# wusize/CLIPSelf

Measured on AMD Instinct MI355X. Metric: images/sec (student+teacher distill step), ViT-B/16 32 crops/img, higher is better.
Workload: dtype bf16; 1 GPU; EVA02-CLIP-B-16 CLIPSelf image-patches step, 64 images x 32 crops per GPU, 224^2 (BASELINE configs[1]); global_batch=64, crops_per_image=32, image_size=224, parallelism=dp1, teacher_chunk=2048, teacher_last_block=cls_query_only, teacher_schedule=one_batch_ahead_on_side_stream

## Files before the change

clipself_amd/csrc/attention.hip:

```cpp
#include <type_traits>
#include "cs_common.h"
#include "../../include/clipself_hip.h"
#include <cstdlib>

namespace {

constexpr int HD = 64;
constexpr float LOG2E = 1.4426950408889634f;


#define Z16 (f32x16{0.f, 0.f, 0.f, 0.f, 0.f, 0.f, 0.f, 0.f, 0.f, 0.f, 0.f, 0.f, 0.f, 0.f, 0.f, 0.f})
__device__ __forceinline__ f32x16 zero16() {
    f32x16 z;
#pragma unroll
    for (int e = 0; e < 16; ++e) z[e] = 0.f;
    return z;
}

__device__ __forceinline__ void rope8(U128& v, const float* __restrict__ cs, const float* __restrict__ sn) {
    const float4 c0 = *(const float4*)cs, c1 = *(const float4*)(cs + 4);
    const float4 s0 = *(const float4*)sn, s1 = *(const float4*)(sn + 4);
    const float c[8] = {c0.x, c0.y, c0.z, c0.w, c1.x, c1.y, c1.z, c1.w};
    const float s[8] = {s0.x, s0.y, s0.z, s0.w, s1.x, s1.y, s1.z, s1.w};
#pragma unroll
// ... 373 lines not shown
    constexpr int KI = (CHK * 8 + NT - 1) / NT;
    U128 kr[KI], vin[8], qraw[4];
    const __bf16* kbase = p.qkv + C + h * HD;
    const __bf16* vbase = p.qkv + 2 * C + h * HD;
    const int vkb = min(tid, CHK - 1) >> 3, vc = tid & 7;
#pragma unroll
    for (int it = 0; it < KI; ++it) {
        const int idx = min(tid + it * NT, CHK * 8 - 1), tok = min(idx >> 3, last);
        kr[it].u = *(const uint4*)(kbase + (rowbase + tok) * p.ldqkv + (idx & 7) * 8);
    }
#pragma unroll
    for (int i = 0; i < 8; ++i) {
        const int tok = min(vkb * 8 + i, last);
        vin[i].u = *(const uint4*)(vbase + (rowbase + tok) * p.ldqkv + vc * 8);
    }
    const int q0 = wave * 32, q = q0 + l31, qc = min(q, last);
#pragma unroll
    for (int ks = 0; ks < 4; ++ks) qraw[ks].u = *(const uint4*)(p.qkv + (rowbase + qc) * p.ldqkv + h * HD + ks * 16 + hf * 8);
    if constexpr (ROPE) {
        if (tid < p.grid * 32) {
            rt[tid] = tab[0];
            rt[(p.grid << 5) + tid] = tab[1];
            rt[(2 * p.grid << 5) + tid] = tab[2];
            rt[(3 * p.grid << 5) + tid] = tab[3];
        }
        __syncthreads();
    }
#pragma unroll
    for (int it = 0; it < KI; ++it) {
        const int idx = tid + it * NT, r = idx >> 3, c = idx & 7;
        if (idx < CHK * 8) {
// ... 19 lines not shown
        if (ROPE && qc > 0 && !ATT_ABL(p, 2)) rope8_lds(qraw[ks], rt, p.grid, p.inv_grid, qc, ks * 2 + hf);
        qf[ks] = qraw[ks].h;
    }
    float m = -INFINITY, l = 0.f;
    f32x16 o[2] = {zero16(), zero16()};
    if (ATT_ABL(p, 1)) { l = 1.f; m = 0.f; o[0][0] = bf2f(qf[0][0]); }
    else if (TAIL) {
        attend_chunk<3, false, false, !ROPE>(Kl, Vt, qf, 0, p.Ntok, sl2, lane, true, m, l, o, 0);
        attend_chunk<3, false, false, !ROPE>(Kl, Vt, qf, 96, p.Ntok, sl2, lane, false, m, l, o, 3);
        attend_chunk<1, true, false, !ROPE>(Kl, Vt, qf, 192, p.Ntok, sl2, lane, false, m, l, o, 6);
    } else {
        attend_chunk<3, false>(Kl, Vt, qf, 0, p.Ntok, sl2, lane, true, m, l, o, 0);
        if (p.Ntok > 96) attend_chunk<3, false>(Kl, Vt, qf, 96, p.Ntok, sl2, lane, false, m, l, o, 3);
        if (p.Ntok > 192) attend_chunk<1, false>(Kl, Vt, qf, 192, p.Ntok, sl2, lane, false, m, l, o, 6);
    }
    if (q < p.Ntok) store_o(p, rowbase, q, h, bh, hf, m, l, o);
}

__global__ __launch_bounds__(256) void attn_bwd_prep_kernel(const __bf16* __restrict__ o, const __bf16* __restrict__ dout, float* __restrict__ dsum,
                                                            int B, int Ntok, int H, int ldo) {
    const long idx = (long)blockIdx.x * blockDim.x + threadIdx.x;
    const long total = (long)B * Ntok * H * 8;
    float s = 0.f;
    long row = 0; int h = 0;
    const bool ok = idx < total;
    if (ok) {
        const int c = (int)(idx & 7);
        h = (int)((idx >> 3) % H);
        row = (idx >> 3) / H;
        U128 a, g;
        a.u = *(const uint4*)(o + row * ldo + h * HD + c * 8);
// ... 1091 lines not shown
```

clipself_amd/csrc/gemm.hip:

```cpp
#include "gemm_common.h"
#include "../../include/clipself_hip.h"
#include <hip/amd_detail/amd_hip_unsafe_atomics.h>

namespace {

constexpr int EP_LD = 68;
constexpr int EP_BYTES = 32 * EP_LD * 4;

template <int FM, int BN>
__device__ __forceinline__ void epilogue_swiglu(const GemmArgs& p, const f32x16 (&acc)[FM][2], char* slab_bytes, char* rowst_bytes, int lane,
                                                int row0, int tn, int wn) {
    const int l31 = lane & 31, hf = lane >> 5;
    uint32_t* slab = (uint32_t*)slab_bytes;
    const int hbase = tn * (BN / 2) + wn * 32;
    const int hl = hbase + l31;
    float b1 = 0.f, b2 = 0.f;
    if (p.bias && hl < p.group) { b1 = p.bias[hl]; b2 = p.bias[p.group + hl]; }
    const bool ln = p.ln_mean != nullptr;
    float c1 = 0.f, c2 = 0.f;
    float2* rowst = (float2*)rowst_bytes;
    if (ln) {
        if (hl < p.group) { c1 = p.ln_colsum[hl]; c2 = p.ln_colsum[p.group + hl]; }
        for (int r = lane; r < FM * 32; r += 64) {
            const int row = min(row0 + r, p.M - 1);
// ... 262 lines not shown
                for (int it = 0; it < 8; ++it) {
                    const float a = sum_lanes16(ps[it]), b = sum_lanes16(pq[it]);
                    if (sel == it) { sv = a; qv = b; }
                }
                const int row = row_base + rrow + 4 * sel;
                if (sel < 8 && row < p.M && n0 + wn * 64 < p.N) {
                    const size_t slice = (size_t)tn * (BN / 64) + wn;
                    *(float2*)(p.stats_part + (slice * p.M + row) * 2) = make_float2(sv, qv);
                }
            }
        }
        if (i + 1 < FM) asm volatile("s_waitcnt lgkmcnt(0)" ::: "memory");
    }
}

template <int EPI, int BM, int BN, int WM, int WN, bool GLDS, int NS>
__global__ __launch_bounds__(WM * WN * 64) void gemm_nt_kernel(GemmArgs p) {
    constexpr int NW = WM * WN;
    constexpr int TM = BM / WM, TN = BN / WN;
    constexpr int FM = TM / 32, FN = TN / 32;
    constexpr int A_BYTES = BM * BK * 2, B_BYTES = BN * BK * 2, STAGE = A_BYTES + B_BYTES;
    constexpr int A_INSTR = BM / 8 / NW, B_INSTR = BN / 8 / NW;
    extern __shared__ __attribute__((aligned(16))) char smem[];

    const int tid = threadIdx.x;
    const int lane = tid & 63;
    const int wave = __builtin_amdgcn_readfirstlane(tid >> 6);
    const int wm = wave / WN, wn = wave - wm * WN;
    const int hf = lane >> 5, l31 = lane & 31;
    int tm, tn;
    tile_of_block(p, tm, tn);
    const int m0 = tm * BM, n0 = tn * BN;

    int arow[A_INSTR], achk[A_INSTR], brow[B_INSTR], bchk[B_INSTR];
    source_rows<EPI, BM, BN, NW, A_INSTR, B_INSTR>(p, wave, lane, m0, n0, tn, arow, achk, brow, bchk);

    const int kt_begin = blockIdx.y * p.ktiles_per_split;
    const int kt_end = min(kt_begin + p.ktiles_per_split, p.K / BK);

    f32x16 acc[FM][FN];
#pragma unroll
    for (int i = 0; i < FM; ++i)
#pragma unroll
        for (int j = 0; j < FN; ++j)
#pragma unroll
            for (int e = 0; e < 16; ++e) acc[i][j][e] = 0.f;

    constexpr bool AB = (NS == 32);
    char* const b_ring = smem + 3 * A_BYTES;
    if (kt_begin < kt_end) {
        stage_tile<A_INSTR, GLDS>(p.A, p.lda, kt_begin * BK, smem, wave * A_INSTR, lane, arow, achk);
        stage_tile<B_INSTR, GLDS>(p.B, p.ldb, kt_begin * BK, AB ? b_ring : smem + A_BYTES, wave * B_INSTR, lane, brow, bchk);
    }
    if (AB && kt_begin + 1 < kt_end)
        stage_tile<A_INSTR, GLDS>(p.A, p.lda, (kt_begin + 1) * BK, smem + A_BYTES, wave * A_INSTR, lane, arow, achk);
    const int a_base = ((wm * TM + l31) >> 1) << 8;
    const int b_base = ((wn * TN + l31) >> 1) << 8;
    const int par8 = (l31 & 1) << 3, sw = l31 >> 1;
    int cur = 0;
    for (int kt = kt_begin; kt < kt_end; ++kt) {
        if (AB) {
            if (kt + 1 < kt_end) asm volatile("s_waitcnt vmcnt(%0)" ::"n"(A_INSTR) : "memory");
            else asm volatile("s_waitcnt vmcnt(0)" ::: "memory");
            asm volatile("s_waitcnt lgkmcnt(0)" ::: "memory");
            __builtin_amdgcn_s_barrier();
            const int i = kt - kt_begin;
            if (!(A_INSTR == 4 && B_INSTR == 4) || (p.dbg & 8)) {
                if (kt + 1 < kt_end)
                    stage_tile<B_INSTR, GLDS>(p.B, p.ldb, (kt + 1) * BK, b_ring + ((i + 1) & 1) * B_BYTES, wave * B_INSTR, lane, brow, bchk);
                if (kt + 2 < kt_end)
                    stage_tile<A_INSTR, GLDS>(p.A, p.lda, (kt + 2) * BK, smem + ((i + 2) % 3) * A_BYTES, wave * A_INSTR, lane, arow, achk);
            }
        } else {
            __syncthreads();
            if (kt + 1 < kt_end && !CS_ABL(p, 1)) {
                char* nxt = smem + (cur ^ 1) * STAGE;
                stage_tile<A_INSTR, GLDS>(p.A, p.lda, (kt + 1) * BK, nxt, wave * A_INSTR, lane, arow, achk);
                stage_tile<B_INSTR, GLDS>(p.B, p.ldb, (kt + 1) * BK, nxt + A_BYTES, wave * B_INSTR, lane, brow, bchk);
            }
        }
        const char* la = (AB ? smem + cur * A_BYTES : smem + cur * STAGE) + a_base;
        const char* lb = (AB ? b_ring + ((kt - kt_begin) & 1) * B_BYTES : smem + cur * STAGE + A_BYTES) + b_base;
        if (CS_ABL(p, 2)) { cur = AB ? (cur == 2 ? 0 : cur + 1) : (cur ^ 1); continue; }
#pragma unroll
        for (int ks = 0; ks < 4; ++ks) {
            const int off = ((par8 | (ks * 2 + hf)) ^ sw) << 4;
            bf16x8 a[FM], b[FN];
#pragma unroll
            for (int i = 0; i < FM; ++i) a[i] = *(const bf16x8*)(la + i * (16 * 256) + off);
#pragma unroll
            for (int j = 0; j < FN; ++j) b[j] = *(const bf16x8*)(lb + j * (16 * 256) + off);
            if (AB && A_INSTR == 4 && B_INSTR == 4 && !(p.dbg & 8)) {
                const int i0 = kt - kt_begin;
#pragma unroll
                for (int h2 = 0; h2 < 2; ++h2) {
                    const int x = (ks & 1) * 2 + h2;
                    if (ks < 2) {
                        if (kt + 1 < kt_end) {
                            const int r1[1] = {brow[x]}, c1[1] = {bchk[x]};
                            stage_tile<1, GLDS>(p.B, p.ldb, (kt + 1) * BK, b_ring + ((i0 + 1) & 1) * B_BYTES, wave * B_INSTR + x, lane, r1, c1);
                        }
                    } else if (kt + 2 < kt_end) {
                        const int r1[1] = {arow[x]}, c1[1] = {achk[x]};
                        stage_tile<1, GLDS>(p.A, p.lda, (kt + 2) * BK, smem + ((i0 + 2) % 3) * A_BYTES, wave * A_INSTR + x, lane, r1, c1);
                    }
                }
            }
#pragma unroll
            for (int i = 0; i < FM; ++i)
#pragma unroll
                for (int j = 0; j < FN; ++j) acc[i][j] = __builtin_amdgcn_mfma_f32_32x32x16_bf16(a[i], b[j], acc[i][j], 0, 0, 0);
        }
        cur = AB ? (cur == 2 ? 0 : cur + 1) : (cur ^ 1);
    }
    __syncthreads();
    if (CS_ABL(p, 4)) return;
    epilogue<EPI, FM, FN, BN>(p, acc, smem, wave, lane, m0 + wm * TM, n0, tn, wn);
}

template <int EPI, int RM = 0>
__global__ __launch_bounds__(512) void gemm_persist_kernel(GemmArgs p) {
    constexpr int AUX_A = RM == 2 ? 2 : 0, AUX_B = RM == 3 ? 2 : 0;
    constexpr bool BSTAT = RM == 1 || RM == 2;
    static_assert(epi_is_bf16(EPI) || EPI == EPI_SWIGLU_BF16 || EPI == EPI_RESID_F32 || EPI == EPI_RESID_LN_F32, "epilogues whose slabs fit");
    constexpr bool PACKED = epi_is_bf16(EPI) || EPI == EPI_SWIGLU_BF16;
    constexpr int BM = 256, BN = 256, WN = 4, NW = 8, TM = 128, TN = 64, FM = 4, FN = 2;
// ... 80 lines not shown
            if (more) tile_of_id(p, next, ntiles, tm, tn);
        }
        if (more) {
            source_rows<EPI, BM, BN, NW, A_INSTR, B_INSTR>(p, wave, lane, tm * BM, tn * BN, tn, arow, achk, brow, bchk);
            prologue();
        }
        if constexpr (EPI == EPI_SWIGLU_BF16) epilogue_swiglu<FM, BN>(p, acc, slab, rowst, lane, m0 + wm * TM, tn_cur, wn);
        else if constexpr (epi_is_bf16(EPI)) epilogue_bf16<FM, BN, epi_act(EPI)>(p, acc, slab, rowst, lane, m0 + wm * TM, n0, wn);
        else epilogue_at<EPI, FM, FN, BN, 64>(p, acc, slab, lane, m0 + wm * TM, n0, tn_cur, wn);
        if (!more) break;
        tile = next;
        first = false;
    }
}

template <int EPI, int BM, int BN, int WM, int WN, int NS>
int launch_cfg(GemmArgs a, int splits, int use_glds, hipStream_t stream) {
    a.tiles_m = (a.M + BM - 1) / BM;
    a.tiles_n = (EPI == EPI_SWIGLU_BF16) ? (a.group + BN / 2 - 1) / (BN / 2) : (a.N + BN - 1) / BN;
    constexpr int NW = WM * WN;
    constexpr size_t stage = NS == 32 ? (size_t)(3 * BM + 2 * BN) * BK * 2 : (size_t)(BM + BN) * BK * 2 * NS;
    constexpr size_t lds = stage > (size_t)NW * EP_BYTES ? stage : (size_t)NW * EP_BYTES;
    dim3 grid(a.tiles_m * a.tiles_n, splits), block(NW * 64);
    if (use_glds) {
        static bool once = ((void)hipFuncSetAttribute((const void*)gemm_nt_kernel<EPI, BM, BN, WM, WN, true, NS>,
                                                      hipFuncAttributeMaxDynamicSharedMemorySize, (int)lds), true);
        (void)once;
        hipLaunchKernelGGL((gemm_nt_kernel<EPI, BM, BN, WM, WN, true, NS>), grid, block, lds, stream, a);
    } else {
        static bool once = ((void)hipFuncSetAttribute((const void*)gemm_nt_kernel<EPI, BM, BN, WM, WN, false, NS>,
                                                      hipFuncAttributeMaxDynamicSharedMemorySize, (int)lds), true);
        (void)once;
        hipLaunchKernelGGL((gemm_nt_kernel<EPI, BM, BN, WM, WN, false, NS>), grid, block, lds, stream, a);
    }
    CS_LAUNCH_CHECK();
    return 0;
}

template <int EPI, int RM>
// ... 11 lines not shown
    constexpr int BM = 256, BN = 256;
    a.tiles_m = (a.M + BM - 1) / BM;
    a.tiles_n = (EPI == EPI_SWIGLU_BF16) ? (a.group + BN / 2 - 1) / (BN / 2) : (a.N + BN - 1) / BN;
    const long ntiles = (long)a.tiles_m * a.tiles_n;
    const long cap = cs_persistent_cap(a.reserve);
    const unsigned grid = (unsigned)(ntiles < cap ? ntiles : cap);
    if constexpr (EPI == EPI_BF16 || EPI == EPI_SWIGLU_BF16) {
        const bool parts_ok = (long)grid == cap && grid % 8 == 0 && a.tiles_n >= a.nsplit && a.tiles_m >= 8 / a.nsplit;
        if (a.rm == 1 && parts_ok) return launch_persist_rm<EPI, 1>(a, grid, stream);
        if (a.rm == 2 && parts_ok) return launch_persist_rm<EPI, 2>(a, grid, stream);
        if (a.rm == 3) return launch_persist_rm<EPI, 3>(a, grid, stream);
    }
    return launch_persist_rm<EPI, 0>(a, grid, stream);
}

template <int EPI>
int launch(GemmArgs a, int splits, int use_glds, int force_cfg, hipStream_t stream) {
    const long ncols = (EPI == EPI_SWIGLU_BF16) ? 2L * a.group : a.N;
    const int ktiles = a.K / BK;
    auto tiles = [&](int bm, int bn) { return (long)((a.M + bm - 1) / bm) * ((ncols + bn - 1) / bn); };
    const double out_bytes = 4.0 * (double)a.M * (double)ncols;
    auto best_split = [&](int bm, int bn, int per_cu, double us_per_ktile, double& cost) {
        const long t = tiles(bm, bn);
        const long slots = (long)cs_num_cus() * per_cu;
        int best = 1;
        cost = 1e30;
        const int lo = splits > 0 ? splits : 1, hi = splits > 0 ? splits : (ktiles < 64 ? ktiles : 64);
        for (int s = lo; s <= hi; ++s) {
            const long rounds = (t * s + slots - 1) / slots;
            const int kper = (ktiles + s - 1) / s;
            const double c = rounds * (kper * us_per_ktile + 5.0) + (EPI == EPI_ATOMIC_F32 ? s * out_bytes / 0.33e6 : 0.0);
            if (c < cost) { cost = c; best = s; }
        }
        return best;
    };
    double c1, c2, c3;
    const int sp[4] = {0, best_split(128, 128, 2, 1.3, c1), best_split(256, 128, 1, 0.95, c2), best_split(256, 256, 1, 1.4, c3)};
    int cfg = force_cfg;
    if (cfg == 0) {
        if (a.M < 256 || ncols < 256) c3 = 1e30;
        if (a.M < 256 || ncols < 128) c2 = 1e30;
        cfg = (c3 <= c2 && c3 <= c1) ? 3 : (c2 <= c1 ? 2 : 1);
        if (cfg == 3 && use_glds) cfg = 11;
    }
    if (cfg != 1 && cfg != 2 && cfg != 3 && cfg != 7 && cfg != 9 && cfg != 11) {
        cs_set_error("cs_gemm_nt: schedule %d does not exist (flags bits 4-7: 0 heuristic, 1, 2, 3, 7, 9, 11)", cfg);
        return -1;
    }
    const int ns = sp[cfg >= 7 ? 3 : cfg];
    a.ktiles_per_split = (ktiles + ns - 1) / ns;
    if (cfg == 11) {
        if (use_glds && ns == 1) {
            const int rc = cs_gemm_stream_launch(a, EPI, a.reserve, stream);
            if (rc <= 0) return rc;
        }
        cfg = 9;
    }
    switch (cfg) {
        case 9:
            if constexpr (epi_is_bf16(EPI) || EPI == EPI_SWIGLU_BF16 || EPI == EPI_RESID_F32 || EPI == EPI_RESID_LN_F32) {
                if (use_glds && ns == 1) return launch_persist<EPI>(a, stream);
            }
            return launch_cfg<EPI, 256, 256, 2, 4, 32>(a, ns, use_glds, stream);
        case 7: return launch_cfg<EPI, 256, 256, 2, 4, 32>(a, ns, use_glds, stream);
        case 3: return launch_cfg<EPI, 256, 256, 2, 4, 2>(a, ns, use_glds, stream);
        case 2: return launch_cfg<EPI, 256, 128, 4, 2, 2>(a, ns, use_glds, stream);
        default: return launch_cfg<EPI, 128, 128, 2, 2, 2>(a, ns, use_glds, stream);
    }
}

__global__ __launch_bounds__(256) void splitk_reduce_act_kernel(const float* __restrict__ ws, int splits, long stride,
                                                                const float* __restrict__ bias, __bf16* __restrict__ C, int M, int N,
                                                                int ldc, int relu) {
    const long i = (long)blockIdx.x * 256 + threadIdx.x;
    const int n4 = N >> 2;
    if (i >= (long)M * n4) return;
    const int row = (int)(i / n4), c = (int)(i - (long)row * n4) * 4;
    const float* src = ws + (size_t)row * N + c;
    float4 acc = *(const float4*)src;
    for (int s = 1; s < splits; ++s) {
        const float4 t = *(const float4*)(src + (size_t)s * stride);
        acc.x += t.x; acc.y += t.y; acc.z += t.z; acc.w += t.w;
// ... 10 lines not shown
}

constexpr int SPLITK_MAX = 8, SPLITK_MIN_KTILES = 16;
int choose_bf16_splits(int M, int N, int K) {
    const long tiles = (long)((M + 255) / 256) * ((N + 255) / 256);
    const int ktiles = K / BK;
    int s = 1;
    while (s < SPLITK_MAX && tiles * (s * 2) <= cs_num_cus() && ktiles / (s * 2) >= SPLITK_MIN_KTILES) s *= 2;
    return s;
}

}

static int gemm_nt_split_f32(const void* A, const void* B, float* C, int M, int N, int K, int lda, int ldb, int cfg, int splits, hipStream_t stream);

static int gemm_nt_impl(const void* A, const void* B, void* C, const float* bias, const float* extra, const float* ln_mean,
                        const float* ln_rstd, const float* ln_colsum, float* stats_part, void* xb_out, int ldxb, int M, int N, int K, int lda,
                        int ldb, int ldc, int epi, int splits, int group, int flags, hipStream_t stream) {
    if (epi == EPI_THIN_FWD || epi == EPI_THIN_DGRAD) {
        CS_CHECK_ARG(!ln_mean && !ln_rstd && !ln_colsum && !stats_part && !xb_out, "cs_gemm_nt_ln: epilogue %d takes no folded LayerNorm", epi);
        return cs_thin_launch(A, B, C, bias, extra, M, N, K, lda, ldb, ldc, epi, splits, group, flags, stream);
    }
    CS_CHECK_ARG(M > 0 && N > 0 && K > 0, "cs_gemm_nt: empty problem M=%d N=%d K=%d", M, N, K);
    CS_CHECK_ARG(K % BK == 0, "cs_gemm_nt: K=%d must be a multiple of %d", K, BK);
    CS_CHECK_ARG((lda % 8) == 0 && (ldb % 8) == 0, "cs_gemm_nt: lda/ldb must be multiples of 8 (16-byte rows)");
    CS_CHECK_ARG(((uintptr_t)A % 16) == 0 && ((uintptr_t)B % 16) == 0, "cs_gemm_nt: operands must be 16-byte aligned");
    const bool splitk_bf16 = (epi == EPI_BF16 || epi == EPI_RELU_BF16) && ln_mean == nullptr;
    CS_CHECK_ARG(splits == 1 || epi == EPI_ATOMIC_F32 || splitk_bf16,
                 "cs_gemm_nt: split-K (splits != 1; <= 0 = automatic) exists for epilogues 0 and 9 (through a workspace) and 4 (atomic), not %d", epi);
    CS_CHECK_ARG((epi == EPI_SWIGLU_BF16 ? group : N) % 4 == 0 && ldc % 4 == 0 && ((uintptr_t)C % 16) == 0,
                 "cs_gemm_nt: N, ldc must be multiples of 4 and C 16-byte aligned (vector epilogue)");
    CS_CHECK_ARG(bias == nullptr || ((uintptr_t)bias % 16) == 0, "cs_gemm_nt: bias must be 16-byte aligned");
    if (splitk_bf16 && splits != 1) {
        const int ns = splits > 0 ? splits : choose_bf16_splits(M, N, K);
        CS_CHECK_ARG(ns <= K / BK, "cs_gemm_nt: splits=%d exceeds the %d K tiles of K=%d", ns, K / BK, K);
        if (ns > 1) {
// ... 325 lines not shown
```

clipself_amd/csrc/gemm_common.h:

```cpp
#pragma once
#include "cs_common.h"
#include <cstdio>
#include <cstdlib>
#include <type_traits>

#ifdef CS_ABLATION_SWITCHES
#define CS_ABL(p, bit) ((p).dbg & (bit))
#else
#define CS_ABL(p, bit) false
#endif

constexpr int BK = 64;
enum Epi { EPI_BF16 = 0, EPI_F32 = 1, EPI_RESID_F32 = 2, EPI_SWIGLU_BF16 = 3, EPI_ATOMIC_F32 = 4, EPI_PATCH_F32 = 5, EPI_RESID_LN_F32 = 6,
           EPI_GELU_BF16 = 7, EPI_QGELU_BF16 = 8, EPI_RELU_BF16 = 9, EPI_THIN_FWD = 10, EPI_THIN_DGRAD = 11 };
constexpr bool epi_is_bf16(int e) { return e == EPI_BF16 || e == EPI_GELU_BF16 || e == EPI_QGELU_BF16 || e == EPI_RELU_BF16; }
constexpr int epi_act(int e) { return e == EPI_GELU_BF16 ? 1 : (e == EPI_QGELU_BF16 ? 2 : (e == EPI_RELU_BF16 ? 3 : 0)); }

struct GemmArgs {
    const __bf16* A;
    const __bf16* B;
    void* C;
    const float* bias;
    const float* extra;
    int M, N, K;
    int lda, ldb, ldc;
    int tiles_m, tiles_n;
    int ktiles_per_split;
    long split_stride;
    int group;
    int gm;
    int rm;
    int nsplit;
    const float* ln_mean;
    const float* ln_rstd;
    const float* ln_colsum;
    float* stats_part;
    __bf16* xb_out;
    int ldxb;
    unsigned short* lo = nullptr;
    int split = 0;
    int reserve;
    int dbg;
};

inline int cs_num_cus() {
    static const int n = [] {
        int dev = 0, v = 0;
        if (hipGetDevice(&dev) != hipSuccess || hipDeviceGetAttribute(&v, hipDeviceAttributeMultiprocessorCount, dev) != hipSuccess || v <= 0) v = 256;
        return v;
    }();
    return n;
}
inline long cs_persistent_cap(int reserve) {
    const int n = cs_num_cus();
    return n - (reserve > 0 && reserve <= n - 8 ? reserve : 0);
// ... 80 lines not shown
```

clipself_amd/engine.py:

```python
from __future__ import annotations

import math
import os

import torch

from .config import TowerCfg
from .engine_base import (ALIGN, BF16, DX_BF16, DX_F32_ACCUM, DX_F32_ASSIGN, EPI_ATOMIC_F32, EPI_BF16, EPI_F32, EPI_GELU_BF16,
                          EPI_PATCH_F32, EPI_QGELU_BF16, EPI_RESID_F32, EPI_RESID_LN_F32, EPI_SWIGLU_BF16, F32, TowerEngine, _round_up,
                          is_no_decay, padded_hidden)


def param_groups_layout(cfg: TowerCfg, prefix: str = "visual."):
    C, Hd, E, p = cfg.width, cfg.hidden, cfg.embed_dim, cfg.patch_size
    Hp, Kp = padded_hidden(cfg), _round_up(3 * p * p, 64)
    t = lambda name, shape, storage=None: (name, shape, storage if storage is not None else shape)
    groups = [[t(prefix + "cls_token", (1, 1, C))], [t(prefix + "pos_embed", (1, cfg.tokens, C))],
              [t(prefix + "patch_embed.proj.weight", (C, 3, p, p), (C, Kp))], [t(prefix + "patch_embed.proj.bias", (C,))]]
    for i in range(cfg.layers):
        b = f"{prefix}{EvaEngine.BLOCK_TAG}{i}."
        groups += [
            [t(b + "norm1.weight", (C,))], [t(b + "norm1.bias", (C,))],
            [t(b + "attn.q_proj.weight", (C, C)), t(b + "attn.k_proj.weight", (C, C)), t(b + "attn.v_proj.weight", (C, C))],
            [t(b + "attn.q_bias", (C,)), t(b + "attn._k_bias_zero", (C,)), t(b + "attn.v_bias", (C,))],
# ... 172 lines not shown
            half = self.cfg.head_width // 2
            freqs = 1.0 / (10000.0 ** (torch.arange(0, half, 2)[: half // 2].float() / half))
            t = torch.arange(grid).float() / grid * self.cfg.pt_hw_seq_len
            ang = (t[:, None] * freqs[None, :]).repeat_interleave(2, dim=-1)
            full = torch.cat([ang[:, None, :].expand(grid, grid, half), ang[None, :, :].expand(grid, grid, half)], dim=-1)
            full = full.reshape(grid * grid, self.cfg.head_width)
            self._tables[key] = (full.cos().contiguous().to(self.device), full.sin().contiguous().to(self.device))
        return self._tables[key]

    def _stem(self, images, keep=None):
        ops, cfg, P = self.ops, self.cfg, self.prefix
        B, _, S, _ = images.shape
        p, C = cfg.patch_size, cfg.width
        g = S // p
        N, Kpe = g * g + 1, self.Kpe
        A = ops.empty((B * g * g, Kpe), BF16)
        ops.im2row(images.contiguous(), A, p)
        x = ops.empty((B, N, C), F32)
        pos = self.pos_for(g)
        ops.gemm_nt(A, self.storage_of(self.shadow, P + "patch_embed.proj.weight"), x.view(B * N, C),
                    bias=self.p[P + "patch_embed.proj.bias"], extra=pos, epi=EPI_PATCH_F32, group=g * g)
        ops.cls_row(x, self.p[P + "cls_token"].view(C), pos)
        if keep is not None:
            keep["patches"] = A
        return x, g

    def _stacked(self, buf, name, i):
        o, st = self.offsets[self._b(i) + name]
        n = self.STACKED[name]
        return buf[o:o + n * math.prod(st)].view(n * st[0], *st[1:])

    def _qkv_operands(self, i):
        return self._stacked(self.shadow, "attn.q_proj.weight", i), self._stacked(self.master, "attn.q_bias", i)

    def _w12(self, i):
        return self._stacked(self.shadow, "mlp.w1.weight", i), self._stacked(self.master, "mlp.w1.bias", i)

    def _block_linears(self, i):
        b = self._b(i)
# ... 185 lines not shown
```

clipself_amd/engine_base.py:

```python
from __future__ import annotations

import math
import os
from collections import OrderedDict

import torch
import torch.nn.functional as F

from .config import TowerCfg

BF16, F32 = torch.bfloat16, torch.float32
EPI_BF16, EPI_F32, EPI_RESID_F32, EPI_SWIGLU_BF16, EPI_ATOMIC_F32, EPI_PATCH_F32, EPI_RESID_LN_F32, EPI_GELU_BF16, EPI_QGELU_BF16 = range(9)
DX_BF16, DX_F32_ASSIGN, DX_F32_ACCUM = range(3)
ALIGN = 64


def _round_up(x: int, m: int) -> int:
    return (x + m - 1) // m * m


def padded_hidden(cfg: TowerCfg) -> int:
    return _round_up(cfg.hidden, 64)


# ... 109 lines not shown
        self.sync_shadow()
        return missing

    def sync_shadow(self):
        self.ops.cast_f32_bf16(self.master, self.shadow)
        self._pos_cache.clear()
        self.block_fold_ratio = None
        if self.trainable or self.HEAD_FWD_TRANSPOSED:
            self.sync_transposed()
        if self._wants_folds():
            self._build_folds()

    def _wants_folds(self) -> bool:
        return self.fold_block_ln

    def _wt_alloc(self, key, rows, cols):
        t = self.wt.get(key)
        if t is None:
            t = self.ops.zeros((cols, _round_up(rows, 64)), BF16)
            self.wt[key] = t
        return t

    def _block_wt_pairs(self, blocks=None):
        blocks = range(self.first_trainable, self.cfg.layers) if blocks is None else blocks
        return [(W, self._wt_alloc((i, key), *W.shape)) for i in blocks for key, W in self._block_linears(i)]

    def set_trainable_blocks(self, unlocked_groups: int):
        L = self.cfg.layers
        self.first_trainable = L - unlocked_groups if 0 < unlocked_groups <= L else 0
        self.train_all = False
# ... 428 lines not shown
```

clipself_amd/engine_openai.py:

```python
from __future__ import annotations

import os

import torch

from .config import TowerCfg
from .engine_base import (BF16, DX_F32_ACCUM, DX_F32_ASSIGN, EPI_BF16, EPI_F32, EPI_GELU_BF16, EPI_PATCH_F32, EPI_QGELU_BF16,
                          EPI_RESID_F32, F32, TowerEngine, _round_up)


def clip_vit_layout(cfg: TowerCfg, prefix: str = "visual."):
    C, Hd, E, p = cfg.width, cfg.hidden, cfg.embed_dim, cfg.patch_size
    Kp = _round_up(3 * p * p, 64)
    t = lambda name, shape, storage=None: (name, shape, storage if storage is not None else shape)
    groups = [[t(prefix + "class_embedding", (C,))], [t(prefix + "positional_embedding", (cfg.tokens, C))],
              [t(prefix + "conv1.weight", (C, 3, p, p), (C, Kp))], [t(prefix + "ln_pre.weight", (C,))], [t(prefix + "ln_pre.bias", (C,))]]
    for i in range(cfg.layers):
        b = f"{prefix}{ClipVitEngine.BLOCK_TAG}{i}."
        groups += [[t(b + "ln_1.weight", (C,))], [t(b + "ln_1.bias", (C,))],
                   [t(b + "attn.in_proj_weight", (3 * C, C))], [t(b + "attn.in_proj_bias", (3 * C,))],
                   [t(b + "attn.out_proj.weight", (C, C))], [t(b + "attn.out_proj.bias", (C,))],
                   [t(b + "ln_2.weight", (C,))], [t(b + "ln_2.bias", (C,))],
                   [t(b + "mlp.c_fc.weight", (Hd, C))], [t(b + "mlp.c_fc.bias", (Hd,))],
                   [t(b + "mlp.c_proj.weight", (C, Hd))], [t(b + "mlp.c_proj.bias", (C,))]]
# ... 118 lines not shown
    def rope_tables(self, grid: int):
        if getattr(self.ops, "ATTN_NO_ROPE", False) and os.environ.get("CLIPSELF_ATTN_IDENTITY_ROPE", "0") in ("", "0"):
            return None, None
        key = ("rope", grid)
        if key not in self._tables:
            shape = (grid * grid, self.cfg.head_width)
            self._tables[key] = (torch.ones(shape, dtype=F32, device=self.device), torch.zeros(shape, dtype=F32, device=self.device))
        return self._tables[key]

    def _stem(self, images, keep=None):
        ops, cfg, P = self.ops, self.cfg, self.prefix
        B, _, S, _ = images.shape
        p, C = cfg.patch_size, cfg.width
        g = S // p
        N = g * g + 1
        A = ops.empty((B * g * g, self.Kpe), BF16)
        ops.im2row(images.contiguous(), A, p)
        x = ops.empty((B, N, C), F32)
        pos = self.pos_for(g)
        ops.gemm_nt(A, self.storage_of(self.shadow, P + "conv1.weight"), x.view(B * N, C), extra=pos, epi=EPI_PATCH_F32, group=g * g)
        ops.cls_row(x, self.p[P + "class_embedding"], pos)
        y = ops.empty((B, N, C), F32)
        mean = rstd = None
        if keep is not None:
            mean, rstd = ops.empty((B * N,), F32), ops.empty((B * N,), F32)
            keep.update(patches=A, x_pre=x.view(B * N, C), st=(mean, rstd))
        ops.layernorm_fwd_f32(x.view(B * N, C), self.p[P + "ln_pre.weight"], self.p[P + "ln_pre.bias"], y.view(B * N, C), mean, rstd, cfg.ln_eps)
        return y, g

    def _block_tail(self, i, x, att, save=None, inplace=True):
        return block_fwd_mlp(self.ops, self.p, self.w, self._b(i), self.cfg.ln_eps, self.cfg.quick_gelu, x, att, save, inplace)

    def _block_fwd(self, i, x, B, N, cos, sin, with_attn=True, save=None, inplace=True):
        ops, cfg = self.ops, self.cfg
        C, H, eps = cfg.width, cfg.heads, cfg.ln_eps
# ... 258 lines not shown
```

clipself_amd/hip.py:

```python
from __future__ import annotations

import ctypes
import os
import subprocess
from pathlib import Path

import torch

_CSRC = Path(__file__).resolve().parent / "csrc"
_LIB_PATH = Path(os.environ["CLIPSELF_HIP_LIB"]) if os.environ.get("CLIPSELF_HIP_LIB") else _CSRC / "libclipself_hip.so"

EPI_BF16, EPI_F32, EPI_RESID_F32, EPI_SWIGLU_BF16, EPI_ATOMIC_F32, EPI_PATCH_F32, EPI_RESID_LN_F32, EPI_GELU_BF16, EPI_QGELU_BF16 = range(9)
EPI_RELU_BF16 = 9
EPI_THIN_FWD, EPI_THIN_DGRAD = 10, 11
THIN_MAX_N = 16
SPLITK_MAX, SPLITK_MIN_KTILES = 8, 16
DX_BF16, DX_F32_ASSIGN, DX_F32_ACCUM = range(3)
ADAMW_GUARD_HEAD, ADAMW_GUARD_SPAN = 8, 16384

_vp, _i, _l, _f, _sz = ctypes.c_void_p, ctypes.c_int, ctypes.c_long, ctypes.c_float, ctypes.c_size_t
_F32, _F32_BF16 = (torch.float32,), (torch.float32, torch.bfloat16)

SIGNATURES = {
    "cs_last_error": (ctypes.c_char_p, []),
    "cs_gemm_nt": (_i, [_vp, _vp, _vp, _vp, _vp, _i, _i, _i, _i, _i, _i, _i, _i, _i, _i, _vp]),
    "cs_crop_resize_workspace": (_sz, [_i, _i, _i]),
    "cs_crop_resize_u8": (_i, [_vp, _i, _i, _vp, _i, _i, _i, _vp, _vp, _vp, _vp, _vp]),
    "cs_quant_rows_fp8": (_i, [_vp, _l, _vp, _l, _vp, _i, _i, _vp]),
    "cs_gemm_nt_f8": (_i, [_vp, _vp, _vp, _vp, _vp, _vp, _vp, _i, _i, _i, _i, _i, _i, _i, _i, _vp]),
# ... 207 lines not shown
    ADAMW_GUARD = True
    ATTN_NO_ROPE = True
    TOKEN_TAPS = True
    DECONV_ROWS = True
    DET_POST = True
    ROI_EXTRACT = True
    ASSIGN = True
    LOSS = True
    MASK = True
    RPN = True
    CONV3X3 = True
    BATCHNORM = True
    LINEAR_ACT = True
    FPN_TOPDOWN = True
    THIN_HEADS = True
    BOX_SCORES = True

    def __init__(self):
        self.lib = load_library()
        if not torch.cuda.is_available():
            raise RuntimeError("HipOps needs a ROCm device (torch.cuda.is_available() is False); no CPU fallback exists")
        self.gemm_flags = 0
        self._rccl_reserve = 0
        self._share = 0
        self._cap = 0
        self.num_cus = int(self.lib.cs_num_compute_units())

    def _update_flags(self):
        n = self._rccl_reserve + self._share
        if self._cap:
# ... 558 lines not shown

    def colsum_bf16(self, x, out, workspace=None):
        self._chk(x, out, workspace)
        M, N = x.shape
        need = self.colsum_workspace(M, N)
        if workspace is None or workspace.numel() * workspace.element_size() < need:
            workspace = torch.empty(need, dtype=torch.uint8, device=x.device)
        self._ok(self.lib.cs_colsum_bf16(_p(x), x.stride(0), _p(out), _p(workspace), M, N, self._stream()), "cs_colsum_bf16")

    def im2row(self, img, out, p):
        self._chk(img, out)
        B, _, S, _ = img.shape
        assert img.is_contiguous()
        assert out.stride(1) == 1 and out.stride(0) == out.shape[1], "im2row writes whole rows (zeros in [3*p*p, ldo)): out must be contiguous"
        self._ok(self.lib.cs_im2row(_p(img), _dt(img), _p(out), B, S, p, out.stride(0), self._stream()), "cs_im2row")

    def cls_row(self, x, cls, pos):
        self._chk(x, cls, pos)
        B, Ntok, C = x.shape
        self._ok(self.lib.cs_cls_row(_p(x), _p(cls), _p(pos), B, Ntok, C, self._stream()), "cs_cls_row")

    @staticmethod
    def _token_map(feat, grid_h, grid_w, tok_off):
        E = feat.shape[-1]
        assert feat.dtype == torch.float32 and feat.stride(-1) == 1 and E % 4 == 0 and feat.stride(0) % E == 0 and feat.data_ptr() % 16 == 0
        if feat.dim() == 4:
            assert tuple(feat.shape[1:3]) == (grid_h, grid_w) and feat.stride(2) == E and feat.stride(1) == grid_w * E, \
                "a [B, h, w, E] map must be a view of the token-major layout"
        else:
            assert feat.dim() == 3 and feat.stride(1) == E
# ... 605 lines not shown
```

Baseline: 749.2 images/sec.

## Fuse im2row into patch-embed GEMM via implicit image A-operand loads

The patch-embedding GEMM now gathers its A operand straight from the image tensor (fp32 or bf16), rounds it to bf16 in registers and writes it to LDS. This replaces the separate im2row kernel and its materialised bf16 patch matrix whenever backward does not need the patches kept. It removes one kernel launch and a round trip of the patch matrix through memory, but A now goes through register loads instead of the DMA path and forgoes schedule 11. A separate change adds an ablation flag to the attention kernel that makes one wave recompute queries redundantly without storing them.

```diff
diff --git a/clipself_amd/csrc/attention.hip b/clipself_amd/csrc/attention.hip
--- a/clipself_amd/csrc/attention.hip
+++ b/clipself_amd/csrc/attention.hip
@@ -411,7 +411,8 @@
         const int tok = min(vkb * 8 + i, last);
         vin[i].u = *(const uint4*)(vbase + (rowbase + tok) * p.ldqkv + vc * 8);
     }
-    const int q0 = wave * 32, q = q0 + l31, qc = min(q, last);
+    const bool redundant = ATT_ABL(p, 8) && wave == 7;
+    const int q0 = redundant ? 0 : wave * 32, q = q0 + l31, qc = min(q, last);
 #pragma unroll
     for (int ks = 0; ks < 4; ++ks) qraw[ks].u = *(const uint4*)(p.qkv + (rowbase + qc) * p.ldqkv + h * HD + ks * 16 + hf * 8);
     if constexpr (ROPE) {
@@ -461,7 +462,7 @@
         if (p.Ntok > 96) attend_chunk<3, false>(Kl, Vt, qf, 96, p.Ntok, sl2, lane, false, m, l, o, 3);
         if (p.Ntok > 192) attend_chunk<1, false>(Kl, Vt, qf, 192, p.Ntok, sl2, lane, false, m, l, o, 6);
     }
-    if (q < p.Ntok) store_o(p, rowbase, q, h, bh, hf, m, l, o);
+    if (q < p.Ntok && !redundant) store_o(p, rowbase, q, h, bh, hf, m, l, o);
 }
 
 __global__ __launch_bounds__(256) void attn_bwd_prep_kernel(const __bf16* __restrict__ o, const __bf16* __restrict__ dout, float* __restrict__ dsum,
diff --git a/clipself_amd/csrc/gemm.hip b/clipself_amd/csrc/gemm.hip
--- a/clipself_amd/csrc/gemm.hip
+++ b/clipself_amd/csrc/gemm.hip
@@ -300,8 +300,52 @@
     }
 }
 
-template <int EPI, int BM, int BN, int WM, int WN, bool GLDS, int NS>
+template <int IMG>
+struct PatchRun {
+    uint4 v[IMG == 1 ? 2 : 1];
+};
+
+__device__ __forceinline__ int patch_row_base(const GemmArgs& p, int row, int img0) {
+    const int b = row / p.group, t = row - b * p.group;
+    const int py = t / p.img_g, px = t - py * p.img_g;
+    return (((b - img0) * 3 * p.lda + (py << p.img_lp)) * p.lda) + (px << p.img_lp);
+}
+
+template <int IMG>
+__device__ __forceinline__ void patch_fetch(const GemmArgs& p, const void* img, int base, int k, bool live, PatchRun<IMG>& r) {
+    const int pm = (1 << p.img_lp) - 1;
+    const int c = k >> (2 * p.img_lp), iy = (k >> p.img_lp) & pm, ix = k & pm;
+    const int off = live ? base + (c * p.lda + iy) * p.lda + ix : 0;
+    if (IMG == 1) {
+        const uint4* s = (const uint4*)((const float*)img + off);
+        r.v[0] = s[0];
+        r.v[1] = s[1];
+    } else {
+        r.v[0] = *(const uint4*)((const __bf16*)img + off);
+    }
+}
+
+template <int IMG>
+__device__ __forceinline__ uint4 patch_round(const PatchRun<IMG>& r) {
+    U128 o;
+    if (IMG == 1) {
+        union { uint4 u[2]; float f[8]; } s;
+        s.u[0] = r.v[0];
+        s.u[1] = r.v[1];
+#pragma unroll
+        for (int e = 0; e < 8; ++e) o.e[e] = f2bf(s.f[e]);
+    } else {
+        U128 s;
+        s.u = r.v[0];
+#pragma unroll
+        for (int e = 0; e < 8; ++e) o.e[e] = f2bf((float)s.e[e]);
+    }
+    return o.u;
+}
+
+template <int EPI, int BM, int BN, int WM, int WN, bool GLDS, int NS, int IMG = 0>
 __global__ __launch_bounds__(WM * WN * 64) void gemm_nt_kernel(GemmArgs p) {
+    static_assert(IMG == 0 || (EPI == EPI_PATCH_F32 && GLDS), "the implicit A operand belongs to the patch embedding; B keeps the DMA");
     constexpr int NW = WM * WN;
     constexpr int TM = BM / WM, TN = BN / WN;
     constexpr int FM = TM / 32, FN = TN / 32;
@@ -320,6 +364,23 @@
 
     int arow[A_INSTR], achk[A_INSTR], brow[B_INSTR], bchk[B_INSTR];
     source_rows<EPI, BM, BN, NW, A_INSTR, B_INSTR>(p, wave, lane, m0, n0, tn, arow, achk, brow, bchk);
+    int abase[A_INSTR];
+    PatchRun<IMG> arun[A_INSTR];
+    const void* img = nullptr;
+    if constexpr (IMG != 0) {
+        const int img0 = min(m0, p.M - 1) / p.group;
+        img = (const char*)p.A + (size_t)img0 * 3 * p.lda * p.lda * (IMG == 1 ? 4 : 2);
+#pragma unroll
+        for (int i = 0; i < A_INSTR; ++i) abase[i] = patch_row_base(p, arow[i], img0);
+    }
+    auto a_fetch = [&](int kt, bool live) {
+#pragma unroll
+        for (int i = 0; i < A_INSTR; ++i) patch_fetch<IMG>(p, img, abase[i], kt * BK + achk[i] * 8, live, arun[i]);
+    };
+    auto a_store = [&](char* tile) {
+#pragma unroll
+        for (int i = 0; i < A_INSTR; ++i) *(uint4*)(tile + (wave * A_INSTR + i) * 1024 + lane * 16) = patch_round<IMG>(arun[i]);
+    };
 
     const int kt_begin = blockIdx.y * p.ktiles_per_split;
     const int kt_end = min(kt_begin + p.ktiles_per_split, p.K / BK);
@@ -333,35 +394,41 @@
             for (int e = 0; e < 16; ++e) acc[i][j][e] = 0.f;
 
     constexpr bool AB = (NS == 32);
+    constexpr int AHEAD = AB ? 2 : 1;
     char* const b_ring = smem + 3 * A_BYTES;
     if (kt_begin < kt_end) {
-        stage_tile<A_INSTR, GLDS>(p.A, p.lda, kt_begin * BK, smem, wave * A_INSTR, lane, arow, achk);
+        if constexpr (IMG != 0) { a_fetch(kt_begin, true); a_store(smem); }
+        else stage_tile<A_INSTR, GLDS>(p.A, p.lda, kt_begin * BK, smem, wave * A_INSTR, lane, arow, achk);
         stage_tile<B_INSTR, GLDS>(p.B, p.ldb, kt_begin * BK, AB ? b_ring : smem + A_BYTES, wave * B_INSTR, lane, brow, bchk);
     }
-    if (AB && kt_begin + 1 < kt_end)
-        stage_tile<A_INSTR, GLDS>(p.A, p.lda, (kt_begin + 1) * BK, smem + A_BYTES, wave * A_INSTR, lane, arow, achk);
+    if (AB && kt_begin + 1 < kt_end) {
+        if constexpr (IMG != 0) { a_fetch(kt_begin + 1, true); a_store(smem + A_BYTES); }
+        else stage_tile<A_INSTR, GLDS>(p.A, p.lda, (kt_begin + 1) * BK, smem + A_BYTES, wave * A_INSTR, lane, arow, achk);
+    }
     const int a_base = ((wm * TM + l31) >> 1) << 8;
     const int b_base = ((wn * TN + l31) >> 1) << 8;
     const int par8 = (l31 & 1) << 3, sw = l31 >> 1;
     int cur = 0;
     for (int kt = kt_begin; kt < kt_end; ++kt) {
         if (AB) {
-            if (kt + 1 < kt_end) asm volatile("s_waitcnt vmcnt(%0)" ::"n"(A_INSTR) : "memory");
+            if (IMG == 0 && kt + 1 < kt_end) asm volatile("s_waitcnt vmcnt(%0)" ::"n"(A_INSTR) : "memory");
             else asm volatile("s_waitcnt vmcnt(0)" ::: "memory");
             asm volatile("s_waitcnt lgkmcnt(0)" ::: "memory");
             __builtin_amdgcn_s_barrier();
             const int i = kt - kt_begin;
+            if constexpr (IMG != 0) a_fetch(kt + 2, kt + 2 < kt_end);
             if (!(A_INSTR == 4 && B_INSTR == 4) || (p.dbg & 8)) {
                 if (kt + 1 < kt_end)
                     stage_tile<B_INSTR, GLDS>(p.B, p.ldb, (kt + 1) * BK, b_ring + ((i + 1) & 1) * B_BYTES, wave * B_INSTR, lane, brow, bchk);
-                if (kt + 2 < kt_end)
+                if (IMG == 0 && kt + 2 < kt_end)
                     stage_tile<A_INSTR, GLDS>(p.A, p.lda, (kt + 2) * BK, smem + ((i + 2) % 3) * A_BYTES, wave * A_INSTR, lane, arow, achk);
             }
         } else {
             __syncthreads();
+            if constexpr (IMG != 0) a_fetch(kt + 1, kt + 1 < kt_end);
             if (kt + 1 < kt_end && !CS_ABL(p, 1)) {
                 char* nxt = smem + (cur ^ 1) * STAGE;
-                stage_tile<A_INSTR, GLDS>(p.A, p.lda, (kt + 1) * BK, nxt, wave * A_INSTR, lane, arow, achk);
+                if constexpr (IMG == 0) stage_tile<A_INSTR, GLDS>(p.A, p.lda, (kt + 1) * BK, nxt, wave * A_INSTR, lane, arow, achk);
                 stage_tile<B_INSTR, GLDS>(p.B, p.ldb, (kt + 1) * BK, nxt + A_BYTES, wave * B_INSTR, lane, brow, bchk);
             }
         }
@@ -386,7 +453,7 @@
                             const int r1[1] = {brow[x]}, c1[1] = {bchk[x]};
                             stage_tile<1, GLDS>(p.B, p.ldb, (kt + 1) * BK, b_ring + ((i0 + 1) & 1) * B_BYTES, wave * B_INSTR + x, lane, r1, c1);
                         }
-                    } else if (kt + 2 < kt_end) {
+                    } else if (IMG == 0 && kt + 2 < kt_end) {
                         const int r1[1] = {arow[x]}, c1[1] = {achk[x]};
                         stage_tile<1, GLDS>(p.A, p.lda, (kt + 2) * BK, smem + ((i0 + 2) % 3) * A_BYTES, wave * A_INSTR + x, lane, r1, c1);
                     }
@@ -396,6 +463,9 @@
             for (int i = 0; i < FM; ++i)
 #pragma unroll
                 for (int j = 0; j < FN; ++j) acc[i][j] = __builtin_amdgcn_mfma_f32_32x32x16_bf16(a[i], b[j], acc[i][j], 0, 0, 0);
+        }
+        if constexpr (IMG != 0) {
+            if (kt + AHEAD < kt_end) a_store(AB ? smem + ((kt - kt_begin + 2) % 3) * A_BYTES : smem + (cur ^ 1) * STAGE);
         }
         cur = AB ? (cur == 2 ? 0 : cur + 1) : (cur ^ 1);
     }
@@ -506,7 +576,7 @@
     }
 }
 
-template <int EPI, int BM, int BN, int WM, int WN, int NS>
+template <int EPI, int BM, int BN, int WM, int WN, int NS, int IMG = 0>
 int launch_cfg(GemmArgs a, int splits, int use_glds, hipStream_t stream) {
     a.tiles_m = (a.M + BM - 1) / BM;
     a.tiles_n = (EPI == EPI_SWIGLU_BF16) ? (a.group + BN / 2 - 1) / (BN / 2) : (a.N + BN - 1) / BN;
@@ -514,7 +584,12 @@
     constexpr size_t stage = NS == 32 ? (size_t)(3 * BM + 2 * BN) * BK * 2 : (size_t)(BM + BN) * BK * 2 * NS;
     constexpr size_t lds = stage > (size_t)NW * EP_BYTES ? stage : (size_t)NW * EP_BYTES;
     dim3 grid(a.tiles_m * a.tiles_n, splits), block(NW * 64);
-    if (use_glds) {
+    if constexpr (IMG != 0) {
+        static bool once = ((void)hipFuncSetAttribute((const void*)gemm_nt_kernel<EPI, BM, BN, WM, WN, true, NS, IMG>,
+                                                      hipFuncAttributeMaxDynamicSharedMemorySize, (int)lds), true);
+        (void)once;
+        hipLaunchKernelGGL((gemm_nt_kernel<EPI, BM, BN, WM, WN, true, NS, IMG>), grid, block, lds, stream, a);
+    } else if (use_glds) {
         static bool once = ((void)hipFuncSetAttribute((const void*)gemm_nt_kernel<EPI, BM, BN, WM, WN, true, NS>,
                                                       hipFuncAttributeMaxDynamicSharedMemorySize, (int)lds), true);
         (void)once;
@@ -556,7 +631,7 @@
     return launch_persist_rm<EPI, 0>(a, grid, stream);
 }
 
-template <int EPI>
+template <int EPI, int IMG = 0>
 int launch(GemmArgs a, int splits, int use_glds, int force_cfg, hipStream_t stream) {
     const long ncols = (EPI == EPI_SWIGLU_BF16) ? 2L * a.group : a.N;
     const int ktiles = a.K / BK;
@@ -583,7 +658,7 @@
         if (a.M < 256 || ncols < 256) c3 = 1e30;
         if (a.M < 256 || ncols < 128) c2 = 1e30;
         cfg = (c3 <= c2 && c3 <= c1) ? 3 : (c2 <= c1 ? 2 : 1);
-        if (cfg == 3 && use_glds) cfg = 11;
+        if (cfg == 3 && use_glds && IMG == 0) cfg = 11;
     }
     if (cfg != 1 && cfg != 2 && cfg != 3 && cfg != 7 && cfg != 9 && cfg != 11) {
         cs_set_error("cs_gemm_nt: schedule %d does not exist (flags bits 4-7: 0 heuristic, 1, 2, 3, 7, 9, 11)", cfg);
@@ -603,11 +678,11 @@
             if constexpr (epi_is_bf16(EPI) || EPI == EPI_SWIGLU_BF16 || EPI == EPI_RESID_F32 || EPI == EPI_RESID_LN_F32) {
                 if (use_glds && ns == 1) return launch_persist<EPI>(a, stream);
             }
-            return launch_cfg<EPI, 256, 256, 2, 4, 32>(a, ns, use_glds, stream);
-        case 7: return launch_cfg<EPI, 256, 256, 2, 4, 32>(a, ns, use_glds, stream);
-        case 3: return launch_cfg<EPI, 256, 256, 2, 4, 2>(a, ns, use_glds, stream);
-        case 2: return launch_cfg<EPI, 256, 128, 4, 2, 2>(a, ns, use_glds, stream);
-        default: return launch_cfg<EPI, 128, 128, 2, 2, 2>(a, ns, use_glds, stream);
+            return launch_cfg<EPI, 256, 256, 2, 4, 32, IMG>(a, ns, use_glds, stream);
+        case 7: return launch_cfg<EPI, 256, 256, 2, 4, 32, IMG>(a, ns, use_glds, stream);
+        case 3: return launch_cfg<EPI, 256, 256, 2, 4, 2, IMG>(a, ns, use_glds, stream);
+        case 2: return launch_cfg<EPI, 256, 128, 4, 2, 2, IMG>(a, ns, use_glds, stream);
+        default: return launch_cfg<EPI, 128, 128, 2, 2, 2, IMG>(a, ns, use_glds, stream);
     }
 }
 
@@ -648,12 +723,46 @@
 
 static int gemm_nt_split_f32(const void* A, const void* B, float* C, int M, int N, int K, int lda, int ldb, int cfg, int splits, hipStream_t stream);
 
+static int patch_img_impl(const void* img, const void* B, void* C, const float* bias, const float* pos, int M, int N, int K, int S, int ldb,
+                          int ldc, int splits, int group, int flags, hipStream_t stream) {
+    CS_CHECK_ARG(M > 0 && N > 0 && K > 0 && splits == 1, "cs_gemm_nt: epilogue 14 needs a non-empty problem and splits == 1 (M=%d N=%d K=%d splits=%d)", M, N, K, splits);
+    int g = 1;
+    while ((long)(g + 1) * (g + 1) <= group) ++g;
+    CS_CHECK_ARG(group > 0 && g * g == group && M % group == 0, "cs_gemm_nt: epilogue 14 needs group = g*g patches per image dividing M (group=%d M=%d)", group, M);
+    const int p = S > 0 && S % g == 0 ? S / g : 0;
+    int lp = 0;
+    while ((1 << lp) < p) ++lp;
+    CS_CHECK_ARG(p >= 8 && (1 << lp) == p && K == 3 * p * p,
+                 "cs_gemm_nt: epilogue 14 covers patch sizes 8, 16, 32, ... with K == 3*p*p (lda = image side %d, g=%d, K=%d); others go through cs_im2row", S, g, K);
+    CS_CHECK_ARG((long)256 * 3 * S * S <= 0x7fffffffL, "cs_gemm_nt: epilogue 14 indexes a tile's images with 32 bits: image side %d exceeds 1672", S);
+    CS_CHECK_ARG(ldb % 8 == 0 && ldb >= K && ((uintptr_t)img % 16) == 0 && ((uintptr_t)B % 16) == 0, "cs_gemm_nt: epilogue 14 needs 16-byte aligned image and weight rows");
+    CS_CHECK_ARG(N % 4 == 0 && ldc % 4 == 0 && ldc >= N && ((uintptr_t)C % 16) == 0, "cs_gemm_nt: N, ldc must be multiples of 4 and C 16-byte aligned (vector epilogue)");
+    CS_CHECK_ARG((bias == nullptr || ((uintptr_t)bias % 16) == 0) && pos != nullptr && ((uintptr_t)pos % 16) == 0, "cs_gemm_nt: epilogue 14 needs a 16-byte aligned position table (bias aligned or NULL)");
+    GemmArgs a;
+    a.A = (const __bf16*)img; a.B = (const __bf16*)B; a.C = C; a.bias = bias; a.extra = pos;
+    a.M = M; a.N = N; a.K = K; a.lda = S; a.ldb = ldb; a.ldc = ldc; a.group = group;
+    a.img_g = g; a.img_lp = lp;
+    a.split_stride = 0;
+    a.ln_mean = a.ln_rstd = a.ln_colsum = nullptr; a.stats_part = nullptr; a.xb_out = nullptr; a.ldxb = 0;
+    a.tiles_m = a.tiles_n = 0;
+    a.gm = ((flags >> 8) & 15) ? ((flags >> 8) & 15) : 8;
+    a.rm = 0; a.nsplit = 1; a.dbg = 0;
+    a.reserve = (flags >> 20) & 255;
+    a.ktiles_per_split = K / BK;
+    const int force = (flags >> 4) & 15;
+    return (flags & 1) ? launch<EPI_PATCH_F32, 1>(a, 1, 1, force, stream) : launch<EPI_PATCH_F32, 2>(a, 1, 1, force, stream);
+}
+
 static int gemm_nt_impl(const void* A, const void* B, void* C, const float* bias, const float* extra, const float* ln_mean,
                         const float* ln_rstd, const float* ln_colsum, float* stats_part, void* xb_out, int ldxb, int M, int N, int K, int lda,
                         int ldb, int ldc, int epi, int splits, int group, int flags, hipStream_t stream) {
     if (epi == EPI_THIN_FWD || epi == EPI_THIN_DGRAD) {
         CS_CHECK_ARG(!ln_mean && !ln_rstd && !ln_colsum && !stats_part && !xb_out, "cs_gemm_nt_ln: epilogue %d takes no folded LayerNorm", epi);
         return cs_thin_launch(A, B, C, bias, extra, M, N, K, lda, ldb, ldc, epi, splits, group, flags, stream);
+    }
+    if (epi == EPI_PATCH_IMG_F32) {
+        CS_CHECK_ARG(!ln_mean && !ln_rstd && !ln_colsum && !stats_part && !xb_out, "cs_gemm_nt_ln: epilogue %d takes no folded LayerNorm", epi);
+        return patch_img_impl(A, B, C, bias, extra, M, N, K, lda, ldb, ldc, splits, group, flags, stream);
     }
     CS_CHECK_ARG(M > 0 && N > 0 && K > 0, "cs_gemm_nt: empty problem M=%d N=%d K=%d", M, N, K);
     CS_CHECK_ARG(K % BK == 0, "cs_gemm_nt: K=%d must be a multiple of %d", K, BK);
diff --git a/clipself_amd/csrc/gemm_common.h b/clipself_amd/csrc/gemm_common.h
--- a/clipself_amd/csrc/gemm_common.h
+++ b/clipself_amd/csrc/gemm_common.h
@@ -12,7 +12,7 @@
 
 constexpr int BK = 64;
 enum Epi { EPI_BF16 = 0, EPI_F32 = 1, EPI_RESID_F32 = 2, EPI_SWIGLU_BF16 = 3, EPI_ATOMIC_F32 = 4, EPI_PATCH_F32 = 5, EPI_RESID_LN_F32 = 6,
-           EPI_GELU_BF16 = 7, EPI_QGELU_BF16 = 8, EPI_RELU_BF16 = 9, EPI_THIN_FWD = 10, EPI_THIN_DGRAD = 11 };
+           EPI_GELU_BF16 = 7, EPI_QGELU_BF16 = 8, EPI_RELU_BF16 = 9, EPI_THIN_FWD = 10, EPI_THIN_DGRAD = 11, EPI_PATCH_IMG_F32 = 14 };
 constexpr bool epi_is_bf16(int e) { return e == EPI_BF16 || e == EPI_GELU_BF16 || e == EPI_QGELU_BF16 || e == EPI_RELU_BF16; }
 constexpr int epi_act(int e) { return e == EPI_GELU_BF16 ? 1 : (e == EPI_QGELU_BF16 ? 2 : (e == EPI_RELU_BF16 ? 3 : 0)); }
 
@@ -39,6 +39,7 @@
     int ldxb;
     unsigned short* lo = nullptr;
     int split = 0;
+    int img_g = 0, img_lp = 0;
     int reserve;
     int dbg;
 };
diff --git a/clipself_amd/engine.py b/clipself_amd/engine.py
--- a/clipself_amd/engine.py
+++ b/clipself_amd/engine.py
@@ -210,15 +210,18 @@
         p, C = cfg.patch_size, cfg.width
         g = S // p
         N, Kpe = g * g + 1, self.Kpe
-        A = ops.empty((B * g * g, Kpe), BF16)
-        ops.im2row(images.contiguous(), A, p)
         x = ops.empty((B, N, C), F32)
         pos = self.pos_for(g)
-        ops.gemm_nt(A, self.storage_of(self.shadow, P + "patch_embed.proj.weight"), x.view(B * N, C),
-                    bias=self.p[P + "patch_embed.proj.bias"], extra=pos, epi=EPI_PATCH_F32, group=g * g)
+        W, bias = self.storage_of(self.shadow, P + "patch_embed.proj.weight"), self.p[P + "patch_embed.proj.bias"]
+        if keep is None and self._implicit_stem(p):
+            ops.patch_embed(images.contiguous(), W, x, bias, pos, p)
+        else:
+            A = ops.empty((B * g * g, Kpe), BF16)
+            ops.im2row(images.contiguous(), A, p)
+            ops.gemm_nt(A, W, x.view(B * N, C), bias=bias, extra=pos, epi=EPI_PATCH_F32, group=g * g)
+            if keep is not None:
+                keep["patches"] = A
         ops.cls_row(x, self.p[P + "cls_token"].view(C), pos)
-        if keep is not None:
-            keep["patches"] = A
         return x, g
 
     def _stacked(self, buf, name, i):
diff --git a/clipself_amd/engine_base.py b/clipself_amd/engine_base.py
--- a/clipself_amd/engine_base.py
+++ b/clipself_amd/engine_base.py
@@ -147,6 +147,10 @@
     def _wants_folds(self) -> bool:
         return self.fold_block_ln
 
+    def _implicit_stem(self, p: int) -> bool:
+        ops = self.ops
+        return bool(getattr(ops, "PATCH_EMBED", False)) and ops.patch_embed_covers(p) and self.Kpe == 3 * p * p
+
     def _wt_alloc(self, key, rows, cols):
         t = self.wt.get(key)
         if t is None:
diff --git a/clipself_amd/engine_openai.py b/clipself_amd/engine_openai.py
--- a/clipself_amd/engine_openai.py
+++ b/clipself_amd/engine_openai.py
@@ -156,11 +156,16 @@
         p, C = cfg.patch_size, cfg.width
         g = S // p
         N = g * g + 1
-        A = ops.empty((B * g * g, self.Kpe), BF16)
-        ops.im2row(images.contiguous(), A, p)
         x = ops.empty((B, N, C), F32)
         pos = self.pos_for(g)
-        ops.gemm_nt(A, self.storage_of(self.shadow, P + "conv1.weight"), x.view(B * N, C), extra=pos, epi=EPI_PATCH_F32, group=g * g)
+        W = self.storage_of(self.shadow, P + "conv1.weight")
+        A = None
+        if keep is None and self._implicit_stem(p):
+            ops.patch_embed(images.contiguous(), W, x, None, pos, p)
+        else:
+            A = ops.empty((B * g * g, self.Kpe), BF16)
+            ops.im2row(images.contiguous(), A, p)
+            ops.gemm_nt(A, W, x.view(B * N, C), extra=pos, epi=EPI_PATCH_F32, group=g * g)
         ops.cls_row(x, self.p[P + "class_embedding"], pos)
         y = ops.empty((B, N, C), F32)
         mean = rstd = None
diff --git a/clipself_amd/hip.py b/clipself_amd/hip.py
--- a/clipself_amd/hip.py
+++ b/clipself_amd/hip.py
@@ -13,6 +13,7 @@
 EPI_BF16, EPI_F32, EPI_RESID_F32, EPI_SWIGLU_BF16, EPI_ATOMIC_F32, EPI_PATCH_F32, EPI_RESID_LN_F32, EPI_GELU_BF16, EPI_QGELU_BF16 = range(9)
 EPI_RELU_BF16 = 9
 EPI_THIN_FWD, EPI_THIN_DGRAD = 10, 11
+EPI_PATCH_IMG_F32 = 14
 THIN_MAX_N = 16
 SPLITK_MAX, SPLITK_MIN_KTILES = 8, 16
 DX_BF16, DX_F32_ASSIGN, DX_F32_ACCUM = range(3)
@@ -250,6 +251,7 @@
     LINEAR_ACT = True
     FPN_TOPDOWN = True
     THIN_HEADS = True
+    PATCH_EMBED = True
     BOX_SCORES = True
 
     def __init__(self):
@@ -838,6 +840,23 @@
         assert img.is_contiguous()
         assert out.stride(1) == 1 and out.stride(0) == out.shape[1], "im2row writes whole rows (zeros in [3*p*p, ldo)): out must be contiguous"
         self._ok(self.lib.cs_im2row(_p(img), _dt(img), _p(out), B, S, p, out.stride(0), self._stream()), "cs_im2row")
+
+    @staticmethod
+    def patch_embed_covers(p) -> bool:
+        return p >= 8 and p & (p - 1) == 0
+
+    def patch_embed(self, img, W, x, bias, pos, p, flags=0):
+        self._chk(img, W, x, bias, pos)
+        B, ch, S, S2 = img.shape
+        _, N, C = x.shape
+        g = S // p
+        assert ch == 3 and S == S2 and S == g * p and N == g * g + 1 and x.shape[0] == B and self.patch_embed_covers(p)
+        assert img.is_contiguous() and x.is_contiguous() and x.dtype == torch.float32
+        assert W.dtype == torch.bfloat16 and tuple(W.shape) == (C, 3 * p * p) and W.stride(1) == 1
+        assert pos.dtype == torch.float32 and tuple(pos.shape) == (N, C) and pos.is_contiguous() and (bias is None or bias.numel() == C)
+        fl = ((flags | self.gemm_flags) & ~1) | (1 if _dt(img) == 0 else 0)
+        self._ok(self.lib.cs_gemm_nt(_p(img), _p(W), _p(x), _p(bias), _p(pos), B * g * g, C, 3 * p * p, S, W.stride(0), C, EPI_PATCH_IMG_F32, 1,
+                                     g * g, fl, self._stream()), "cs_gemm_nt (patch embed)")
 
     def cls_row(self, x, cls, pos):
         self._chk(x, cls, pos)
```

Result: no change. 750.6 images/sec, median of 6 (+0.2%).
